# mcveanlab/mccortex

Hardware: AMD Instinct MI355X
Metric: k-mers/s inserted (build), k=31, 50M x 150bp synthetic reads (higher is better)
Workload: dtype u64

## Files before the change

### mccortex_amd/csrc/mcx_api.hip

```cpp
#include <hip/hip_runtime.h>

#include <stdarg.h>
#include <stdio.h>
#include <stdlib.h>
#include <string.h>
#include <cstring>

#include <rocprim/device/device_radix_sort.hpp>
#include <rocprim/device/device_scan.hpp>

#include <algorithm>
#include <array>
#include <cmath>
#include <memory>
#include <vector>
#include <thread>
#include <atomic>
#include <chrono>
#include <mutex>
#include <condition_variable>
#include <functional>

#include "../../include/mcx_gpu.h"
#include "mcx_kernels.h"
// ... 524 lines not shown
      case 2: if (one_) F<2, true>(__VA_ARGS__); else F<2, false>(__VA_ARGS__); break; \
      case 3: if (one_) F<3, true>(__VA_ARGS__); else F<3, false>(__VA_ARGS__); break; \
      default: if (one_) F<4, true>(__VA_ARGS__); else F<4, false>(__VA_ARGS__); break; \
    }                                                                                 \
  } while (0)
#define LAUNCH_W4(W_, KERNEL, ...)                                       \
  do {                                                                   \
    switch (W_) {                                                        \
      case 1: hipLaunchKernelGGL((KERNEL<1>), __VA_ARGS__); break;       \
      case 2: hipLaunchKernelGGL((KERNEL<2>), __VA_ARGS__); break;       \
      case 3: hipLaunchKernelGGL((KERNEL<3>), __VA_ARGS__); break;       \
      default: hipLaunchKernelGGL((KERNEL<4>), __VA_ARGS__); break;      \
    }                                                                    \
  } while (0)
#define NO_WIDE(g, what) do { if ((g) && (g)->W > 2) return fail(MCX_ERR_ARG, what " is not available for k > 63"); } while (0)

struct SpanGuard {
  mcx_graph *g; size_t idx; bool on;
  SpanGuard(mcx_graph *g_, const char *name) : g(g_), idx(0), on(g_ && g_->profile) {
    if (!on) return;
    mcx_graph::Span sp{name, nullptr, nullptr};
    (void)hipEventCreate(&sp.a); (void)hipEventCreate(&sp.b);
    (void)hipEventRecord(sp.a, g->stream);
    idx = g->spans.size();
    g->spans.push_back(sp);
  }
  ~SpanGuard() { if (on) (void)hipEventRecord(g->spans[idx].b, g->stream); }
};

static unsigned cl_grid(const mcx_graph *g, uint64_t items)
{
  return (unsigned)std::max<uint64_t>(1, std::min<uint64_t>((items + 255) / 256, (uint64_t)g->grid));
}
#define GRID_LAUNCH(NAME, ITEMS, ...)                                                            \
  do {                                                                                           \
    SpanGuard sp_(g, #NAME);                                                                     \
    hipLaunchKernelGGL(NAME, dim3(cl_grid(g, ITEMS)), dim3(256), 0, st, __VA_ARGS__);            \
    HIP_TRY(hipGetLastError());                                                                  \
  } while (0)
#define GRID_LAUNCH_W(NAME, ITEMS, ...)                                                          \
  do {                                                                                           \
    SpanGuard sp_(g, #NAME);                                                                     \
    LAUNCH_W4(g->W, NAME, dim3(cl_grid(g, ITEMS)), dim3(256), 0, st, __VA_ARGS__);               \
    HIP_TRY(hipGetLastError());                                                                  \
  } while (0)

static void phase_clock(const char *cmd, const char *what, double &t0)
{
  static const bool on = getenv("MCX_TIMING") != nullptr;
  if (!on) return;
  const double t = now_s();
  fprintf(stderr, "[timing]   %s %8.1f ms  %s\n", cmd, (t - t0) * 1e3, what);
  t0 = t;
}

template <class In> static int device_scan(hipStream_t st, const In *in, uint64_t *out, uint64_t cnt)
{
  size_t tmp_bytes = 0;
  HIP_TRY(rocprim::exclusive_scan(nullptr, tmp_bytes, in, out, (uint64_t)0, cnt, rocprim::plus<uint64_t>(), st));
  DevBuf<uint8_t> tmp;
  HIP_TRY(tmp.alloc(std::max<size_t>(tmp_bytes, 1)));
  HIP_TRY(rocprim::exclusive_scan((void *)tmp.p, tmp_bytes, in, out, (uint64_t)0, cnt, rocprim::plus<uint64_t>(), st));
  HIP_TRY(hipStreamSynchronize(st));
  return MCX_OK;
}
template <class In> static int scan_total(hipStream_t st, const In *in, uint64_t *out, uint64_t cnt, uint64_t *total)
{
  int rc = device_scan(st, in, out, cnt);
  if (rc != MCX_OK) return rc;
  HIP_TRY(hipMemcpy(total, out + cnt - 1, 8, hipMemcpyDeviceToHost));
  return MCX_OK;
}

static int sort_perm_scratch(hipStream_t st, uint64_t m, size_t *tmp_bytes)
{
  HIP_TRY(rocprim::radix_sort_pairs(nullptr, *tmp_bytes, (const uint64_t *)nullptr, (uint64_t *)nullptr, (uint64_t *)nullptr, (uint64_t *)nullptr, m, 0, 64, st));
  return MCX_OK;
}
template <class WordFn>
static int sort_perm_by_words(hipStream_t st, uint64_t m, int W, int top_bits, uint64_t *const keys[2], uint64_t *const perm[2], void *tmp,
                              size_t tmp_bytes, mcx_graph *span, WordFn word, uint64_t **out)
{
  uint64_t *cur = perm[0], *nxt = perm[1];
  for (int w = W - 1; w >= 0; w--) {
    const uint64_t *have = nullptr;
    int rc = word(w, w == W - 1, (const uint64_t *)cur, keys[1], &have);
    if (rc != MCX_OK) return rc;
    auto radix_sort_pass = [&](auto *in) {
      SpanGuard sp(span, "radix_sort_pairs");
      return rocprim::radix_sort_pairs(tmp, tmp_bytes, in, keys[0], cur, nxt, m, 0, w ? 64 : top_bits, st);
    };
    HIP_TRY(have ? radix_sort_pass(have) : radix_sort_pass(keys[1]));
    std::swap(cur, nxt);
  }
  *out = cur;
  return MCX_OK;
}

template <class K> static void allow_lds(K kernel, size_t bytes)
{
  (void)hipFuncSetAttribute(reinterpret_cast<const void *>(kernel), hipFuncAttributeMaxDynamicSharedMemorySize, (int)bytes);
}

static StreamArgs make_args(mcx_graph *g, const StreamLaunch &L)
{
  StreamArgs a;
  a.stream = L.stream; a.code = L.code; a.inv = L.inv; a.nbytes = L.nbytes; a.pos_lo = L.pos_lo; a.pos_hi = L.pos_hi;
  a.tile0 = L.pos_lo / kTile;
  a.ntiles = (L.pos_hi + kTile - 1) / kTile;
  a.k = g->k; a.ctr = g->d_ctr; a.flag = L.flag;
  return a;
}

template <int W, bool ONECOL> static void launch_direct_t(mcx_graph *g, const StreamLaunch &L, int colour)
{
  const StreamArgs a = make_args(g, L);
  const uint64_t nt = a.ntiles > a.tile0 ? a.ntiles - a.tile0 : 0;
  if (!nt) return;
  InsertSink<W, ONECOL> is{g->t, (uint32_t)colour};
  SpanGuard sp(g, "k_stream");
  const dim3 grid((unsigned)std::min<uint64_t>(nt, (uint64_t)g->grid));
  if (a.code) hipLaunchKernelGGL((k_stream<W, ONECOL, true>), grid, dim3(kThreads), 0, g->stream, a, is);
  else hipLaunchKernelGGL((k_stream<W, ONECOL, false>), grid, dim3(kThreads), 0, g->stream, a, is);
}

template <int W, bool ONECOL, bool FULL, int SH, bool PK>
static void launch_bin_stream_pk(mcx_graph *g, const StreamArgs &a, uint64_t nt, int colour, BinSpec bs, BinOut out)
{
  InsertSink<W, ONECOL> is{g->t, (uint32_t)colour};
  static bool once_dev[64] = {false};
  bool &once = once_dev[g->device & 63];
  if (!once) {
    allow_lds(k_stream_bin<W, ONECOL, 512, FULL, SH, PK>, sizeof(BinLds<W, 512, FULL>));
    allow_lds(k_stream_bin<W, ONECOL, 1024, FULL, SH, PK>, sizeof(BinLds<W, 1024, FULL>));
    allow_lds(k_stream_bin<W, ONECOL, kMaxBins, FULL, SH, PK>, sizeof(BinLds<W, kMaxBins, FULL>));
    once = true;
  }
  SpanGuard sp(g, "k_stream_bin");
  if constexpr (W == 1 && !FULL && SH == 0) {
    static const int fc_cap = [] { const char *e = getenv("MCX_STREAM_FC"); return e ? atoi(e) : 0; }();
    if (fc_cap && bs.nlocal <= 512) {
      const dim3 gridf((unsigned)std::min<uint64_t>(nt, (uint64_t)(g->grid_stream ? g->grid_stream : g->grid)));
#define MCX_FC_LAUNCH(CAPV, PRIVV) { \
        static bool once_f[64] = {false}; \
        if (!once_f[g->device & 63]) { allow_lds(k_stream_fc<ONECOL, PK, CAPV, PRIVV>, sizeof(FcLds<CAPV>)); once_f[g->device & 63] = true; } \
        hipLaunchKernelGGL((k_stream_fc<ONECOL, PK, CAPV, PRIVV>), gridf, dim3(kThreads), sizeof(FcLds<CAPV>), g->stream, a, bs, out, is); }
      if (bs.rep >= gridf.x && bs.rep > 8) MCX_FC_LAUNCH(10, true)
      else MCX_FC_LAUNCH(10, false)
#undef MCX_FC_LAUNCH
      return;
    }
    static const bool wide = [] { const char *e = getenv("MCX_STREAM_T"); return !e || atoi(e) == 512; }();
    if (wide && bs.nlocal <= 512) {
      using GeoW = Geo<512, 512 * kPosPerLane>;
      static bool once_w[64] = {false};
      if (!once_w[g->device & 63]) { allow_lds(k_stream_bin<W, ONECOL, 512, FULL, SH, PK, 512>, sizeof(BinLds<W, 512, FULL, GeoW>)); once_w[g->device & 63] = true; }
      const dim3 gridw((unsigned)std::min<uint64_t>((nt + 1) / 2, (uint64_t)(g->grid_stream ? g->grid_stream : g->grid)));
      hipLaunchKernelGGL((k_stream_bin<W, ONECOL, 512, FULL, SH, PK, 512>), gridw, dim3(512), sizeof(BinLds<W, 512, FULL, GeoW>), g->stream, a, bs, out, is);
      return;
    }
  }
  const dim3 grid((unsigned)std::min<uint64_t>(nt, (uint64_t)(g->grid_stream ? g->grid_stream : g->grid)));
  if (bs.nlocal <= 512)
    hipLaunchKernelGGL((k_stream_bin<W, ONECOL, 512, FULL, SH, PK>), grid, dim3(kThreads), sizeof(BinLds<W, 512, FULL>), g->stream, a, bs, out, is);
  else if (bs.nlocal <= 1024)
    hipLaunchKernelGGL((k_stream_bin<W, ONECOL, 1024, FULL, SH, PK>), grid, dim3(kThreads), sizeof(BinLds<W, 1024, FULL>), g->stream, a, bs, out, is);
  else
    hipLaunchKernelGGL((k_stream_bin<W, ONECOL, kMaxBins, FULL, SH, PK>), grid, dim3(kThreads), sizeof(BinLds<W, kMaxBins, FULL>), g->stream, a, bs, out, is);
}

template <int W, bool ONECOL, bool FULL, int SH>
static void launch_bin_stream_t(mcx_graph *g, const StreamLaunch &L, int colour, BinSpec bs, BinOut out)
{
  const StreamArgs a = make_args(g, L);
  const uint64_t nt = a.ntiles > a.tile0 ? a.ntiles - a.tile0 : 0;
  if (!nt) return;
  if (!FULL && a.code) launch_bin_stream_pk<W, ONECOL, FULL, SH, !FULL>(g, a, nt, colour, bs, out);
  else launch_bin_stream_pk<W, ONECOL, FULL, SH, false>(g, a, nt, colour, bs, out);
}

template <int W, bool ONECOL, bool IN_FULL, bool SHARD>
static void launch_bin_tuples_t(mcx_graph *g, TupleIn in, int colour, BinSpec bs, BinOut out)
{
  constexpr bool kWide = W == 1 && !IN_FULL;
  static const bool wide = kWide && [] { const char *e = getenv("MCX_SPLIT_T"); return !e || atoi(e) == 512; }();
  const bool use_wide = wide && bs.nlocal <= 1024;
  const bool use_huge = wide && !use_wide && bs.nlocal <= (uint32_t)kMaxBins;
  const uint64_t tile = use_huge ? 1024 * 16 : use_wide ? 512 * 16 : kTile;
  const uint64_t nchunks = (in.seg_cap + tile - 1) / tile * in.nseg;
  if (!nchunks) return;
  InsertSink<W, ONECOL> is{g->t, (uint32_t)colour};
  using GeoW = Geo<512, 512 * 16>;
  static bool once_dev[64] = {false};
  bool &once = once_dev[g->device & 63];
  if (!once) {
    allow_lds(k_tuples_bin<W, ONECOL, 512, IN_FULL, SHARD>, sizeof(BinLds<W, 512, false>));
    allow_lds(k_tuples_bin<W, ONECOL, 1024, IN_FULL, SHARD>, sizeof(BinLds<W, 1024, false>));
    allow_lds(k_tuples_bin<W, ONECOL, kMaxBins, IN_FULL, SHARD>, sizeof(BinLds<W, kMaxBins, false>));
    if constexpr (kWide) allow_lds(k_tuples_bin<W, ONECOL, 512, IN_FULL, SHARD, 512>, sizeof(BinLds<W, 512, false, GeoW>));
    if constexpr (kWide) allow_lds(k_tuples_bin<W, ONECOL, 1024, IN_FULL, SHARD, 512>, sizeof(BinLds<W, 1024, false, GeoW>));
    if constexpr (kWide) allow_lds(k_tuples_bin<W, ONECOL, kMaxBins, IN_FULL, SHARD, 1024>, sizeof(BinLds<W, kMaxBins, false, Geo<1024, 1024 * 16>>));
    once = true;
  }
  SpanGuard sp(g, "k_tuples_bin");
  const uint64_t gmax = (uint64_t)(g->grid_split ? g->grid_split : g->grid * 4);
  if constexpr (kWide) {
    if (use_huge) {
      using GeoH = Geo<1024, 1024 * 16>;
      const dim3 gridh((unsigned)std::min<uint64_t>(nchunks, g->grid_split ? gmax : gmax / 4));
      hipLaunchKernelGGL((k_tuples_bin<W, ONECOL, kMaxBins, IN_FULL, SHARD, 1024>), gridh, dim3(1024), sizeof(BinLds<W, kMaxBins, false, GeoH>), g->stream, in, bs, out, is, g->d_ctr);
      return;
    }
    if (use_wide) {
      const dim3 gridw((unsigned)std::min<uint64_t>(nchunks, g->grid_split ? gmax : gmax / 2));
      if (bs.nlocal <= 512)
        hipLaunchKernelGGL((k_tuples_bin<W, ONECOL, 512, IN_FULL, SHARD, 512>), gridw, dim3(512), sizeof(BinLds<W, 512, false, GeoW>), g->stream, in, bs, out, is, g->d_ctr);
      else
        hipLaunchKernelGGL((k_tuples_bin<W, ONECOL, 1024, IN_FULL, SHARD, 512>), gridw, dim3(512), sizeof(BinLds<W, 1024, false, GeoW>), g->stream, in, bs, out, is, g->d_ctr);
      return;
    }
  }
  const dim3 grid((unsigned)std::min<uint64_t>(nchunks, gmax));
  if (bs.nlocal <= 512)
    hipLaunchKernelGGL((k_tuples_bin<W, ONECOL, 512, IN_FULL, SHARD>), grid, dim3(kThreads), sizeof(BinLds<W, 512, false>), g->stream, in, bs, out, is, g->d_ctr);
  else if (bs.nlocal <= 1024)
    hipLaunchKernelGGL((k_tuples_bin<W, ONECOL, 1024, IN_FULL, SHARD>), grid, dim3(kThreads), sizeof(BinLds<W, 1024, false>), g->stream, in, bs, out, is, g->d_ctr);
  else
    hipLaunchKernelGGL((k_tuples_bin<W, ONECOL, kMaxBins, IN_FULL, SHARD>), grid, dim3(kThreads), sizeof(BinLds<W, kMaxBins, false>), g->stream, in, bs, out, is, g->d_ctr);
}
template <int W, bool ONECOL> static void launch_bin_region_stream(mcx_graph *g, const StreamLaunch &L, int colour, BinSpec bs, BinOut out)
{
  if (g->t.lbo) launch_bin_stream_t<W, ONECOL, false, 1>(g, L, colour, bs, out);
  else launch_bin_stream_t<W, ONECOL, false, 0>(g, L, colour, bs, out);
}
template <int W, bool ONECOL> static void launch_split_regions(mcx_graph *g, TupleIn in, int colour, BinSpec bs, BinOut out)
{ launch_bin_tuples_t<W, ONECOL, false, false>(g, in, colour, bs, out); }
template <int W, bool ONECOL> static void launch_bin_received(mcx_graph *g, TupleIn in, int colour, BinSpec bs, BinOut out)
{
  if (g->t.lbo) launch_bin_tuples_t<W, ONECOL, true, true>(g, in, colour, bs, out);
  else launch_bin_tuples_t<W, ONECOL, true, false>(g, in, colour, bs, out);
}

static uint64_t *l2_ptr(const mcx_graph *g, uint64_t off)
{
  if (g->l2_hi && off >= g->l2_hi_off) return g->l2_hi + (off - g->l2_hi_off) * g->cap2 * g->W;
  return g->l2_keys + off * g->cap2 * g->W;
}

template <int W, bool ONECOL, bool IDX32> static void launch_lds_insert_k(mcx_graph *g, int colour, uint32_t sub0, uint32_t nsub)
{
  const size_t lds = Sub<W>::kSlots * (W + 1) * 8 + LdsQueue<W>::kTuples * 8 * W;
  static bool once_dev[64] = {false};
  bool &once = once_dev[g->device & 63];
  if (!once) { allow_lds(k_lds_insert<W, ONECOL, IDX32>, lds); once = true; }
  BinOut bins{l2_ptr(g, g->l2_off), nullptr, g->l2_cnt + g->l2_off, g->cap2, nullptr, nullptr, nullptr, 0};
  SpanGuard sp(g, "k_lds_insert");
  hipLaunchKernelGGL((k_lds_insert<W, ONECOL, IDX32>), dim3((unsigned)std::min<uint64_t>(nsub, (uint64_t)(g->grid_insert ? g->grid_insert : g->grid * 4))),
                     dim3(LdsCfg<W>::kThreads), lds, g->stream, g->t, (uint32_t)colour, bins, sub0, nsub, g->d_ctr);
}

template <int W, bool ONECOL> static void launch_lds_insert_t(mcx_graph *g, int colour, uint32_t sub0, uint32_t nsub)
{
  if constexpr (W == 1 && ONECOL) {
    if (g->l2_idx32) return launch_lds_insert_k<W, ONECOL, true>(g, colour, sub0, nsub);
  }
  launch_lds_insert_k<W, ONECOL, false>(g, colour, sub0, nsub);
}

template <int W, bool ONECOL>
static void launch_insert_tuples_t(mcx_graph *g, int colour, const uint64_t *keys, const uint8_t *edges, uint64_t n, uint32_t only_own = 0)
{
  const int grid = (int)std::min<uint64_t>((n + kThreads * kBatch - 1) / (kThreads * kBatch), (uint64_t)g->grid);
  InsertSink<W, ONECOL> s{g->t, (uint32_t)colour};
  SpanGuard sp(g, "k_insert_tuples");
  hipLaunchKernelGGL((k_insert_tuples<W, ONECOL>), dim3(grid), dim3(kThreads), 0, g->stream, s, keys, edges, n, g->d_ctr, only_own);
}

static void free_defer(mcx_graph *g)
{
  (void)hipFree(g->l1_keys); (void)hipFree(g->l1_cnt);
  (void)hipFree(g->l2_base); (void)hipFree(g->l2_hi); (void)hipFree(g->l2_cnt);
  g->l1_keys = g->l2_keys = g->l2_base = g->l2_hi = nullptr; g->l1_cnt = g->l2_cnt = nullptr;
  g->cap1 = g->cap2 = 0;
  g->l2_regions = 0;
  g->set_colour.clear(); g->set_pending.clear();
}

__global__ __launch_bounds__(512) void k_l2_probe(uint64_t *keys, uint64_t cap, uint32_t nregions, uint32_t spb, uint32_t iters,
                                                  uint32_t jit_mask = 0 )
{
  const uint32_t region = blockIdx.x % nregions, blk = blockIdx.x / nregions, nblk = gridDim.x / nregions;
  const uint32_t w = threadIdx.x >> 6, l = threadIdx.x & 63u;
  for (uint32_t it = 0; it < iters; it++)
    for (uint32_t k = 0; k < spb / 32u; k++) {
      const uint32_t front = w * 4u + (l >> 4) + 32u * k;
      const uint32_t seg = region * spb + front;
      const uint64_t jit = ((seg * 0x9E3779B1u) >> 8) & jit_mask & ~15u;
      const uint64_t at = (uint64_t)seg * cap + jit + ((uint64_t)it * nblk + blk) * 16u + (l & 15u);
      if (jit + ((uint64_t)it * nblk + blk) * 16u + 16u <= cap) keys[at] = at;
    }
}

static uint64_t *l2_place(mcx_graph *g, size_t bytes, uint32_t nreg, int tries, float *ms_out)
{
  std::vector<uint64_t *> cand;
  std::vector<float> ms;
  hipEvent_t e0 = nullptr, e1 = nullptr;
  if (tries > 1 && (hipEventCreate(&e0) != hipSuccess || hipEventCreate(&e1) != hipSuccess)) { (void)hipGetLastError(); tries = 1; }
  const uint32_t iters = (uint32_t)std::max<uint64_t>(8, g->cap2 * g->W / 1024);
  for (int i = 0; i < std::max(tries, 1); i++) {
    if (i > 0) {
// ... 4105 lines not shown
```

### mccortex_amd/csrc/mcx_defer.h

```cpp
#pragma once
#include "mcx_kernels.h"

namespace mcx {

enum : int { BIN_OWNER = 0, BIN_GROUP = 1, BIN_SUBLOCAL = 2, BIN_GLOBAL = 3 };

struct BinSpec {
  int mode;
  uint32_t nparts;
  uint32_t nlocal;
  uint32_t rep;
  uint32_t nout;
  uint32_t seg_mod;
  uint32_t lb1;
  uint32_t region0;
};

__device__ __forceinline__ uint32_t out_seg(const BinSpec &bs, uint32_t ob0, uint32_t b)
{
  if (bs.mode == BIN_GLOBAL)
    return ((((b >> bs.lb1) * bs.rep + blockIdx.x % bs.rep) << bs.lb1) | (b & ((1u << bs.lb1) - 1u)));
  return ob0 + b;
}

struct BinOut {
  uint64_t *keys;
  uint8_t *edges;
  unsigned long long *counts;
  uint64_t cap;
  uint64_t *ov_keys;
  uint8_t *ov_edges;
  unsigned long long *ov_counts;
  uint64_t ov_cap;
};

#define MCX_LDS_AS __attribute__((address_space(3)))

#ifdef MCX_PHASES
__device__ unsigned long long g_phase[3][8];
#define MCX_PH_DECL unsigned long long ph_t = wall_clock64(), ph_acc[8] = {0, 0, 0, 0, 0, 0, 0, 0};
#define MCX_PH(i) { const unsigned long long n_ = wall_clock64(); ph_acc[i] += n_ - ph_t; ph_t = n_; }
#define MCX_PH_COUNT ph_acc[7]++;
#define MCX_PH_DUMP(kid) { if (threadIdx.x == 0) for (int i_ = 0; i_ < 8; i_++) atomicAdd(&g_phase[kid][i_], ph_acc[i_]); }
#else
#define MCX_PH_DECL
#define MCX_PH(i)
#define MCX_PH_COUNT
#define MCX_PH_DUMP(kid)
#endif
constexpr int kMaxBins = 2048;
constexpr uint64_t kQMask = (1ull << 56) - 1;

template <int W> __device__ __forceinline__ Kmer<W> tuple_pack(const Kmer<W> &q, uint32_t e)
{
  Kmer<W> t = q;
  t.w[0] |= (uint64_t)e << 56;
  return t;
}
template <int W> __device__ __forceinline__ Kmer<W> tuple_q(const Kmer<W> &t)
{
  Kmer<W> q = t;
  q.w[0] &= kQMask;
  return q;
}

constexpr int kRounds = 2;
constexpr int kStage = kTile / kRounds;

template <int T_, int TILE_, int R_ = kRounds> struct Geo {
  static constexpr int kT = T_, kTileG = TILE_, kRoundsG = R_, kStageG = TILE_ / R_;
};
using Geo256 = Geo<kThreads, kTile>;

template <int W, int NB, bool FULL, class G = Geo256> struct BinLds {
  using geo = G;
  uint64_t skey[G::kStageG * W];
  unsigned long long gbase[NB];
  uint32_t cnt[NB + 64];
  uint32_t rnk[NB + 64];
  uint32_t off[NB + 64];
  uint32_t wsum[G::kT / 64];
  uint16_t sbin[G::kStageG];
  uint8_t se[FULL ? G::kStageG : 16];
};

__device__ __forceinline__ uint32_t tid_now()
{
  uint32_t t = threadIdx.x;
  asm volatile("" : "+v"(t));
  return t;
}

template <int NB, int T = kThreads> struct BinRes { unsigned long long g0[(NB + T - 1) / T]; };

template <class LDS, int NB>
__device__ __forceinline__ void bin_reserve(LDS &L, const BinSpec &bs, const BinOut &out, uint32_t ob0, BinRes<NB, LDS::geo::kT> &res,
                                            bool trash_beyond = false)
{
  constexpr int kT = LDS::geo::kT;
  const int tid = threadIdx.x;
  __syncthreads();
  {
    constexpr int PERB = NB / kT;
    static_assert(NB % kT == 0, "bins per thread");
    uint32_t c[PERB], x = 0;
#pragma unroll
    for (int i = 0; i < PERB; i++) {
      const uint32_t b = (uint32_t)tid * PERB + i;
      c[i] = b < bs.nlocal ? L.cnt[b] : 0;
      x += c[i];
    }
    const uint32_t mine = x;
#pragma unroll
    for (int d = 1; d < 64; d <<= 1) {
      const uint32_t y = __shfl_up(x, d, 64);
      if ((tid & 63) >= d) x += y;
    }
    if ((tid & 63) == 63) L.wsum[tid >> 6] = x;
    __syncthreads();
    uint32_t before = 0, total = 0;
#pragma unroll
    for (int w = 0; w < kT / 64; w++) {
      const uint32_t ws = L.wsum[w];
      if (w < (tid >> 6)) before += ws;
      total += ws;
    }
    uint32_t o = before + x - mine;
#pragma unroll
    for (int i = 0; i < PERB; i++) {
      const uint32_t b = (uint32_t)tid * PERB + i;
      if (b < bs.nlocal) L.off[b] = o;
      o += c[i];
    }
    if (tid < 64) L.off[bs.nlocal + tid] = tid && trash_beyond ? (uint32_t)LDS::geo::kTileG : total;
  }
  __syncthreads();
#pragma unroll
  for (int q = 0; q < (NB + kT - 1) / kT; q++) {
    const uint32_t b = (uint32_t)q * kT + tid;
    res.g0[q] = 0;
    if (b < bs.nlocal) {
      const uint32_t c = L.cnt[b];
      if (c) res.g0[q] = atomicAdd(&out.counts[out_seg(bs, ob0, b)], (unsigned long long)c);
    }
  }
}

constexpr unsigned long long kDstMask = (1ULL << 48) - 1;

template <class LDS, int NB>
__device__ __forceinline__ void bin_commit(LDS &L, const BinSpec &bs, const BinOut &out, uint32_t ob0, const BinRes<NB, LDS::geo::kT> &res)
{
  constexpr int kT = LDS::geo::kT;
#pragma unroll
  for (int q = 0; q < (NB + kT - 1) / kT; q++) {
    const uint32_t b = (uint32_t)q * kT + threadIdx.x;
    if (b < bs.nlocal) {
      const uint32_t o0 = L.off[b], o1 = L.off[b + 1];
      const unsigned long long g0 = res.g0[q];
      const unsigned long long room = out.cap > g0 ? out.cap - g0 : 0;
      const uint32_t lim = o0 + (uint32_t)min((unsigned long long)(o1 - o0), room);
      const unsigned long long dst = ((unsigned long long)out_seg(bs, ob0, b) * out.cap + g0 - o0) & kDstMask;
      L.gbase[b] = dst | ((unsigned long long)lim << 48);
    }
  }
}

template <class LDS> __device__ __forceinline__ uint32_t bin_rank(LDS &L, uint32_t local)
{
  return L.off[local] + atomicAdd(&L.rnk[local], 1u);
}

template <int W, bool FULL, class LDS>
__device__ __forceinline__ void bin_place(LDS &L, int round, uint32_t p, uint32_t local, const Kmer<W> &t, uint32_t e)
{
  constexpr uint32_t kSt = LDS::geo::kStageG;
  if ((int)(p / kSt) != round) return;
  const uint32_t q = p % kSt;
  L.skey[q * W] = t.w[0];
  if (W == 2) L.skey[q * W + 1] = t.w[W - 1];
  L.sbin[q] = (uint16_t)local;
  if (FULL) L.se[q] = (uint8_t)e;
}

template <int W, bool ONECOL, bool FULL, int SH, class LDS>
__device__ __forceinline__ void bin_writeout(LDS &L, int round, const BinSpec &bs, const BinOut &out, uint32_t ob0,
                                             uint32_t region_of_seg, const InsertSink<W, ONECOL> &isink,
                                             uint32_t &novel, uint32_t &full)
{
  __syncthreads();
  const uint32_t n = L.off[bs.nlocal];
  constexpr uint32_t kSt = LDS::geo::kStageG;
  const uint32_t lo = (uint32_t)round * kSt;
  const uint32_t hi = min(n, lo + kSt);
  auto emit = [&](uint32_t p, uint32_t b, unsigned long long gb, uint64_t t0, uint64_t t1) {
    if (p < (uint32_t)(gb >> 48)) {
      const uint64_t at = (gb + p) & kDstMask;
      uint64_t *kd = out.keys + at * W;
      kd[0] = t0;
      if (W == 2) kd[1] = t1;
      if (FULL) out.edges[at] = L.se[p - lo];
    } else if (FULL || bs.mode == BIN_OWNER) {
      full = 2;
    } else {
      Kmer<W> tq;
      tq.w[0] = t0;
      if (W == 2) tq.w[W - 1] = t1;
      const uint32_t e = (uint32_t)(tq.w[0] >> 56);
      const Kmer<W> qq = tuple_q<W>(tq);
      const uint32_t lbq = lbq_of(isink.t);
      if (SH == 2) {
        const Kmer<W> key = key_unquot<W>(qq, lbq, b ^ mix_g(region_mix<W>(qq), lbq));
        const uint32_t owner = b >> bs.lb1;
        const unsigned long long pos = atomicAdd(&out.ov_counts[owner], 1ULL);
        if (pos < out.ov_cap) {
          uint64_t *kd = out.ov_keys + ((uint64_t)owner * out.ov_cap + pos) * W;
          kd[0] = key.w[0];
          if (W == 2) kd[1] = key.w[W - 1];
          out.ov_edges[(uint64_t)owner * out.ov_cap + pos] = (uint8_t)e;
        } else {
          const unsigned long long sp_cap = bs.region0 ? out.ov_counts[bs.nparts + 1] : 0;
          const unsigned long long sp = sp_cap ? atomicAdd(&out.ov_counts[bs.nparts], 1ULL) : 0;
          if (sp < sp_cap) {
            const uint64_t at = (uint64_t)bs.nparts * out.ov_cap + sp;
            uint64_t *kd = out.ov_keys + at * W;
            kd[0] = key.w[0];
            if (W == 2) kd[1] = key.w[W - 1];
            out.ov_edges[at] = (uint8_t)e;
          } else {
            full = 2;
          }
        }
      } else {
        table_mark_written(isink.t);
        table_count_fallback(isink.t);
        const uint32_t region = bs.mode == BIN_GROUP ? b : region_of_seg;
        const Kmer<W> key = key_unquot<W>(qq, lbq, r_of<W>(isink.t, region, qq));
        const uint64_t slot = key_slot<W>(isink.t, key);
        const uint64_t cur = *key_ptr_t<W, ONECOL>(isink.t, slot);
        probe_insert<W, ONECOL>(isink.t, key, slot, cur, 0, e, isink.col, novel, full);
      }
    }
  };
  for (uint32_t p = lo + threadIdx.x; p < hi; p += LDS::geo::kT) {
    const uint32_t q = p - lo;
    const uint32_t b = L.sbin[q];
    emit(p, b, L.gbase[b], L.skey[q * W], W == 2 ? L.skey[q * W + W - 1] : 0);
  }
  if (round + 1 < LDS::geo::kRoundsG) __syncthreads();
}

struct LaneWin { uint32_t a2, a1, a0, r2, r1, r0; };
__device__ __forceinline__ uint32_t pairrev32(uint32_t x)
{
  const uint32_t r = __builtin_bitreverse32(x);
  return ((r >> 1) & 0x55555555u) | ((r & 0x55555555u) << 1);
}
__device__ __forceinline__ LaneWin lane_win(const uint32_t *s_code, uint32_t pl, int k)
{
  LaneWin w;
  w.a2 = s_code[pl >> 4];
  w.a1 = s_code[(pl >> 4) + 1];
  w.a0 = s_code[(pl >> 4) + 2];
  const uint32_t c2 = pairrev32(~w.a0), c1 = pairrev32(~w.a1), c0 = pairrev32(~w.a2);
  const int t = 66 - 2 * k;
  if (t < 32) {
    w.r2 = (c2 << t) | (c1 >> (32 - t));
    w.r1 = (c1 << t) | (c0 >> (32 - t));
    w.r0 = c0 << t;
  } else {
    const uint64_t x = (((uint64_t)c1 << 32) | c0) << (t - 32);
    w.r2 = (uint32_t)(x >> 32);
    w.r1 = (uint32_t)x;
    w.r0 = 0;
  }
  return w;
}

template <int W, bool ONECOL>
__device__ __noinline__ void foreign_insert(const InsertSink<W, ONECOL> &isink, Kmer<W> key, uint32_t e,
                                            uint32_t &novel, uint32_t &full)
{
  table_mark_written(isink.t);
  table_count_foreign(isink.t);
  const uint64_t slot = key_slot<W>(isink.t, key);
  const uint64_t cur = *key_ptr_t<W, ONECOL>(isink.t, slot);
  probe_insert<W, ONECOL>(isink.t, key, slot, cur, 0, e, isink.col, novel, full);
}

template <int W, bool ONECOL, int NB, bool FULL, int SH, bool PK, int T = kThreads>
__global__ __launch_bounds__(T, (W == 1 ? 4 : 3)) void k_stream_bin(StreamArgs a_arg, BinSpec bs, BinOut out_arg,
                                                                  InsertSink<W, ONECOL> isink_arg)
{
  constexpr int H = T / kThreads;
  static_assert(T == kThreads || (T == 2 * kThreads && !FULL), "256 threads, or 512 for packed bins");
  __shared__ uint32_t s_code_h[H][kChunks + 4];
  __shared__ uint32_t s_inv_h[H][kChunks / 2 + 4];
  struct Cold { StreamArgs a; InsertSink<W, ONECOL> isink; };
  __shared__ Cold cold;
  if (threadIdx.x == 0) { cold.a = a_arg; cold.isink = isink_arg; }
  __syncthreads();
  const StreamArgs &a = cold.a;
  const BinOut &out = out_arg;
  const InsertSink<W, ONECOL> &isink = cold.isink;
  const uint64_t a_tile0 = a_arg.tile0, a_ntiles = a_arg.ntiles;
  const uint32_t t_lb1 = isink_arg.t.lb1, t_lbq = isink_arg.t.lb1 + isink_arg.t.lbo, t_part = isink_arg.t.part;
  extern __shared__ __attribute__((aligned(16))) unsigned char dyn_lds[];
  using LDS = BinLds<W, NB, FULL, Geo<T, T * kPosPerLane>>;
  LDS &L = *reinterpret_cast<LDS *>(dyn_lds);

  const int tid0 = threadIdx.x & (kThreads - 1);
  const uint64_t half0 = (uint64_t)(threadIdx.x / kThreads);
  const int k = a_arg.k;
  uint32_t n_kmers = 0, n_contigs = 0, n_novel = 0, full = 0;
  const uint64_t top_mask = (W == 1) ? (~0ULL >> (64 - 2 * k)) : (~0ULL >> (128 - 2 * k));
  const int first_shift = (W == 1) ? (2 * k - 2) : (2 * k - 66);
  const uint32_t ob0 = (blockIdx.x % bs.rep) * bs.nout;

  TileSrc pre;
  pre.a = make_uint4(0, 0, 0, 0); pre.b = make_uint4(0, 0, 0, 0);
  {
    const uint64_t t0 = a_tile0 + (uint64_t)blockIdx.x * H + half0;
    if (t0 < a_ntiles) tile_fetch<PK>(a_arg, t0, tid0, pre);
  }
  MCX_PH_DECL
  for (uint64_t tile_b = a_tile0 + (uint64_t)blockIdx.x * H; tile_b < a_ntiles; tile_b += (uint64_t)gridDim.x * H) {
    const int tid_blk = (int)tid_now();
    const int tid = tid_blk & (kThreads - 1);
    const uint64_t tile = tile_b + (uint64_t)(tid_blk / kThreads);
    const bool have_tile = H == 1 || tile < a_ntiles;
    uint32_t *s_code = s_code_h[H == 1 ? 0 : tid_blk / kThreads];
    uint32_t *s_inv = s_inv_h[H == 1 ? 0 : tid_blk / kThreads];
    MCX_PH(6) MCX_PH_COUNT
    tile_stage<PK>(a_arg, pre, tid, s_code, s_inv);
    for (uint32_t b = tid_blk; b < bs.nlocal + 64; b += T) { L.cnt[b] = 0; L.rnk[b] = 0; }
    if (tid < 4) { s_code[kChunks + tid] = 0; s_inv[kChunks / 2 + tid] = 0xFFFFFFFFu; }
    {
      const uint64_t tn = tile + (uint64_t)gridDim.x * H;
      if (tn < a_ntiles) tile_fetch<PK>(a_arg, tn, tid, pre);
    }
    __syncthreads();
    MCX_PH(0)

    const uint32_t pl = 16u * (uint32_t)(tid + 1);
    const uint64_t Vh = inv_win64(s_inv, pl);
    const uint64_t Vl = (W == 2) ? inv_win64(s_inv, pl + 64) : 0;
    const uint32_t prev_chunk_inv = (s_inv[(pl - 1) >> 5] >> (31 - ((pl - 1) & 31))) & 1u;
    uint32_t range = have_tile ? 0xFFFFu : 0u;
    if (have_tile) {
      const uint64_t plo = a.pos_lo, phi = a.pos_hi, T0 = tile * kTile;
      if (T0 < plo || T0 + kTile > phi) {
        const uint64_t P0 = T0 + 16ull * (uint64_t)tid;
        const int j_lo = plo > P0 ? (int)min((uint64_t)kPosPerLane, plo - P0) : 0;
        const int j_hi = phi > P0 ? (int)min((uint64_t)kPosPerLane, phi - P0) : 0;
        range = ((0x10000u >> j_lo) - 1u) & ~((0x10000u >> j_hi) - 1u);
      }
    }
    uint32_t ok16, nok16, pok16;
    {
      uint64_t Mh = Vh, Ml = Vl;
      for (int c = 1; c < k;) {
        const int s = min(c, k - c);
        if (W == 2) Mh |= (Mh << s) | (Ml >> (64 - s));
        else Mh |= Mh << s;
        if (W == 2) Ml |= Ml << s;
        c += s;
      }
      ok16 = ~(uint32_t)(Mh >> 48) & range;
      const int sh = 112 - k;
      const uint64_t nx = sh >= 64 ? (Vh >> (sh - 64)) : ((Vh << (64 - sh)) | (W == 2 ? (Vl >> sh) : 0));
      nok16 = ~(uint32_t)nx & 0xFFFFu;
      pok16 = ~((prev_chunk_inv << 15) | (uint32_t)(Vh >> 49)) & 0xFFFFu;
    }

    Kmer<W> tk[kPosPerLane];
    uint32_t tle[kPosPerLane];
    const uint32_t trash = bs.nlocal + 1u + ((uint32_t)tid_blk & 31u);
    n_kmers += __popc(ok16);
    n_contigs += __popc(ok16 & ~pok16);
    {
      const uint32_t own = s_code[pl >> 4];
      const uint32_t before = s_code[(pl - 1) >> 4] & 3u;
      const uint32_t lbq = t_lbq;
      const uint32_t qmask = (1u << lbq) - 1u, lmask = (1u << t_lb1) - 1u;
      Kmer<W> fw, rc;
      uint64_t feed;
      LaneWin lw;
      if (W == 1) {
        lw = lane_win(s_code, pl, k);
        feed = code_win64(s_code, pl + (uint32_t)k);
      } else {
        const uint64_t hi = code_win64(s_code, pl), lo = code_win64(s_code, pl + 32);
        const int s = 128 - 2 * k;
        fw.w[0] = hi >> s;
        fw.w[W - 1] = (lo >> s) | (hi << (64 - s));
        rc = revcomp<W>(fw, k);
        feed = code_win64(s_code, pl + (uint32_t)k);
      }
      const uint32_t feed32 = (uint32_t)(feed >> 32);
      uint32_t arr_prev = 0;
      const uint32_t key_sh = 64u - 2u * (uint32_t)k;
      const uint32_t mix_sh = (32u - lbq) & 31u;
#pragma unroll
      for (int j = 0; j < kPosPerLane; j++) {
        const uint32_t prev_nuc = j == 0 ? before : ((own >> (32 - 2 * j)) & 3u);
        const uint32_t nuc_next = (feed32 >> (30 - 2 * j)) & 3u;
        const uint32_t valid = 0u - ((ok16 >> (15 - j)) & 1u);
        const uint32_t nb = (nok16 >> (15 - j)) & 1u, pb = (pok16 >> (15 - j)) & 1u;
        uint32_t o, local;
        Kmer<W> key;
        uint64_t sel = 0;
        if (W == 1) {
          const uint32_t fh = j ? __builtin_amdgcn_alignbit(lw.a2, lw.a1, 32 - 2 * j) : lw.a2;
          const uint32_t fl = j ? __builtin_amdgcn_alignbit(lw.a1, lw.a0, 32 - 2 * j) : lw.a1;
          const uint32_t rh = j < 15 ? __builtin_amdgcn_alignbit(lw.r2, lw.r1, 2 + 2 * j) : lw.r2;
          const uint32_t rl = j < 15 ? __builtin_amdgcn_alignbit(lw.r1, lw.r0, 2 + 2 * j) : lw.r1;
          const uint64_t f = ((uint64_t)fh << 32) | fl, r = ((uint64_t)rh << 32) | rl;
          o = f < r ? 0u : 1u;
          sel = f < r ? f : r;
          key.w[0] = sel >> key_sh;
        } else {
          key = canonical<W>(fw, rc, o);
        }
        const uint32_t o4 = o << 2;
        const uint32_t e = (nb << (nuc_next | o4)) | (pb << ((prev_nuc ^ 7u) ^ o4));
        if (FULL) {
          uint32_t h2;
          kmer_hash<W>(key, 0, &h2);
          local = owner_of(h2, bs.nparts);
          tk[j] = key;
          local = (local & valid) | (trash & ~valid);
          tle[j] = local | (e << 24);
        } else {
          uint32_t G;
          Kmer<W> q;
          if (W == 1) {
            const uint64_t kk = sel >> key_sh;
            q.w[0] = kk >> lbq;
            G = ((uint32_t)kk ^ (region_mix<W>(q) >> mix_sh)) & qmask;
          } else {
            uint32_t r;
            q = key_quot<W>(key, lbq, r);
            G = r ^ mix_g(region_mix<W>(q), lbq);
          }
          local = SH == 1 ? (G & lmask) : G;
          tk[j] = tuple_pack<W>(q, e);
          if (SH == 1 && valid && (G >> t_lb1) != t_part) {
            foreign_insert<W, ONECOL>(isink, key, e, n_novel, full);
            local = trash;
          }
          local = (local & valid) | (trash & ~valid);
          tle[j] = local;
        }
        const uint32_t arr_now = atomicAdd(&L.cnt[local], 1u);
        if (j > 0) { tle[j - 1] |= arr_prev << 12; asm volatile("" : "+v"(tle[j - 1])); }
        arr_prev = arr_now;
        if (j == kPosPerLane - 1) tle[j] |= arr_now << 12;
        if (W == 1) asm volatile("" : "+v"(tle[j]), "+v"(tk[j].w[0]));
        else asm volatile("" : "+v"(tle[j]), "+v"(tk[j].w[0]), "+v"(tk[j].w[W - 1]));
        if (W == 2) {
          fw.w[0] = ((fw.w[0] << 2) | (fw.w[W - 1] >> 62)) & top_mask;
          fw.w[W - 1] = (fw.w[W - 1] << 2) | nuc_next;
          rc.w[W - 1] = (rc.w[W - 1] >> 2) | (rc.w[0] << 62);
          rc.w[0] = (rc.w[0] >> 2) | ((uint64_t)(3u - nuc_next) << first_shift);
        }
      }
    }
    MCX_PH(1)
    BinRes<NB, T> res;
    bin_reserve<LDS, NB>(L, bs, out, ob0, res, !FULL);
    MCX_PH(2)
#pragma unroll
    for (int j = 0; j < kPosPerLane; j++) {
      tle[j] += L.off[tle[j] & 0xfffu] << 12;
      if ((j & 3) == 3) asm volatile("" : "+v"(tle[j - 3]), "+v"(tle[j - 2]), "+v"(tle[j - 1]), "+v"(tle[j]));
    }
    bin_commit<LDS, NB>(L, bs, out, ob0, res);
    MCX_PH(3)
    for (int round = 0; round < kRounds; round++) {
#pragma unroll
      for (int j = 0; j < kPosPerLane; j++)
        bin_place<W, FULL, LDS>(L, round, FULL ? (tle[j] >> 12) & 0xfffu : tle[j] >> 12, tle[j] & 0xfffu, tk[j], tle[j] >> 24);
      bin_writeout<W, ONECOL, FULL, SH, LDS>(L, round, bs, out, ob0, 0, isink, n_novel, full);
      if (round == 0) { MCX_PH(4) } else { MCX_PH(5) }
    }
  }
  MCX_PH_DUMP(0)

  block_add(&a.ctr->kmers, n_kmers);
  block_add(&a.ctr->contigs, n_contigs);
  block_add(&a.ctr->novel, n_novel);
  if (full == 1) a.ctr->full = 1;
  if (full == 2) a.ctr->bin_over = 1;
  if (a.flag && n_contigs) *a.flag = 1;
}

struct TupleIn {
  const uint64_t *keys;
  const uint8_t *edges;
  const unsigned long long *counts;
  uint64_t seg_cap;
  uint32_t nseg;
  uint32_t seg_group, seg_stride;
  uint32_t set_rep;
  uint8_t set_map[32];
};
__device__ __forceinline__ uint64_t tuple_seg_phys(const TupleIn &in, uint32_t seg)
{
  uint32_t q = seg / in.seg_group;
  if (in.set_rep) q = (uint32_t)in.set_map[q / in.set_rep] * in.set_rep + q % in.set_rep;
  return (uint64_t)q * in.seg_stride + seg % in.seg_group;
}

template <int W, bool ONECOL, int NB, bool IN_FULL, bool SHARD, int T = kThreads, int R = kRounds, int P = 16>
__global__ __launch_bounds__(T, (W == 1 || T > kThreads ? 4 : 3)) void k_tuples_bin(TupleIn in, BinSpec bs, BinOut out,
                                                                         InsertSink<W, ONECOL> isink_arg, Counters *ctr)
{
  extern __shared__ __attribute__((aligned(16))) unsigned char dyn_lds[];
  using LDS = BinLds<W, NB, false, Geo<T, T * P, R>>;
  constexpr int kThreads = T, kTile = T * P;
  LDS &L = *reinterpret_cast<LDS *>(dyn_lds);
  __shared__ InsertSink<W, ONECOL> isink;
  if (threadIdx.x == 0) isink = isink_arg;
  __syncthreads();
  const uint32_t t_spb = isink_arg.t.spb, t_lb1 = isink_arg.t.lb1, t_lbq = isink_arg.t.lb1 + isink_arg.t.lbo, t_part = isink_arg.t.part;
  const int tid = threadIdx.x;
  uint32_t n_novel = 0, full = 0;
  const uint64_t chunks_per_seg = (in.seg_cap + kTile - 1) / kTile;
  const bool xcd = bs.mode == BIN_SUBLOCAL && gridDim.x % 8 == 0 && bs.seg_mod % 8 == 0 && in.nseg % bs.seg_mod == 0;
  const uint32_t group = xcd ? blockIdx.x % 8 : 0;
  const uint32_t nseg_g = xcd ? in.nseg / 8 : in.nseg;
  constexpr uint32_t kWin = 2;
  const uint32_t bins_g = xcd ? bs.seg_mod / 8 : 1;
  const uint32_t reps = xcd ? in.nseg / bs.seg_mod : 1;
  const uint32_t win_segs = kWin * reps;
  const uint32_t nwin = (bins_g + kWin - 1) / kWin;
  const uint64_t nchunks = xcd ? (uint64_t)nwin * chunks_per_seg * win_segs : chunks_per_seg * nseg_g;
  const uint64_t v0 = xcd ? blockIdx.x / 8 : blockIdx.x, vstep = xcd ? gridDim.x / 8 : gridDim.x;
  const uint32_t lmask = (1u << t_lb1) - 1u;
  MCX_PH_DECL
  for (uint64_t v = v0; v < nchunks; v += vstep) {
    uint32_t seg;
    uint64_t start;
    if (xcd) {
      const uint64_t per_win = chunks_per_seg * win_segs;
      const uint32_t win = (uint32_t)(v / per_win);
      const uint64_t rem = v % per_win;
      const uint32_t s = (uint32_t)(rem % win_segs);
      const uint32_t rgi = win * kWin + s % kWin;
      if (rgi >= bins_g) continue;
      seg = (s / kWin) * bs.seg_mod + group + 8 * rgi;
      start = (rem / win_segs) * kTile;
    } else {
      seg = (uint32_t)(v % nseg_g);
      start = (v / nseg_g) * kTile;
    }
    const uint64_t pseg = tuple_seg_phys(in, seg);
    uint64_t cnt = in.counts ? (uint64_t)in.counts[pseg] : in.seg_cap;
    if (cnt > in.seg_cap) cnt = in.seg_cap;
    if (start >= cnt) continue;
    const uint32_t n = (uint32_t)min((uint64_t)kTile, cnt - start);
    const uint32_t lregion = bs.mode == BIN_SUBLOCAL ? seg % bs.seg_mod : 0;
    const uint32_t region = bs.region0 + lregion;
    const uint32_t ob0 = (bs.mode == BIN_SUBLOCAL ? lregion * t_spb : 0) + (blockIdx.x % bs.rep) * bs.nout;
    MCX_PH(6) MCX_PH_COUNT
    __syncthreads();
    for (uint32_t b = tid; b < bs.nlocal + 64; b += kThreads) { L.cnt[b] = 0; L.rnk[b] = 0; }
    __syncthreads();
    MCX_PH(0)
    const uint32_t trash = bs.nlocal + 1u + ((uint32_t)tid & 31u);
    const uint64_t *kin = in.keys + (pseg * in.seg_cap + start) * W;
    const uint8_t *ein = IN_FULL ? in.edges + pseg * in.seg_cap + start : nullptr;
    constexpr int PER = kTile / kThreads;
    Kmer<W> tk[PER];
    uint32_t ev[IN_FULL ? PER : 1], loc[PER];
    uint32_t okm = 0;
    const bool vec16 = !IN_FULL && (((uintptr_t)in.keys & 15u) == 0) && (W == 2 || (in.seg_cap & 1u) == 0);
    if (vec16) {
      const ulonglong2 *kin2 = reinterpret_cast<const ulonglong2 *>(kin);
#pragma unroll
      for (int q = 0; q < PER; q += (W == 1 ? 2 : 1)) {
        const uint32_t p = (uint32_t)(q / (W == 1 ? 2 : 1)) * kThreads + tid;
        const uint32_t i = W == 1 ? 2 * p : p;
        tk[q].w[0] = 0; tk[q + (W == 1 ? 1 : 0)].w[W - 1] = 0;
        if (i < n) {
          const ulonglong2 x = kin2[p];
          okm |= 1u << q;
          if (W == 1) {
            tk[q].w[0] = x.x;
            tk[q + (W == 1 ? 1 : 0)].w[0] = x.y;
            if (i + 1 < n) okm |= 2u << q;
          } else {
            tk[q].w[0] = x.x;
            tk[q].w[W - 1] = x.y;
          }
        }
      }
    } else {
#pragma unroll
    for (int q = 0; q < PER; q++) {
      const uint32_t i = (uint32_t)q * kThreads + tid;
      if (i < n) okm |= 1u << q;
      tk[q].w[0] = 0; if (W == 2) tk[q].w[W - 1] = 0;
      if (IN_FULL) ev[q] = 0;
      if (i < n) {
        tk[q].w[0] = kin[(uint64_t)i * W];
        if (W == 2) tk[q].w[W - 1] = kin[(uint64_t)i * W + 1];
        if (IN_FULL) ev[q] = ein[i];
      }
    }
    }
#pragma unroll
    for (int q = 0; q < PER; q++) {
      const uint32_t i = (uint32_t)q * kThreads + tid;
      uint32_t hb;
      if (IN_FULL) {
        uint32_t r;
        const uint32_t lbq = t_lbq;
        const Kmer<W> key = tk[q];
        const Kmer<W> qq = key_quot<W>(key, lbq, r);
        const uint32_t G = r ^ mix_g(region_mix<W>(qq), lbq);
        hb = 0;
        loc[q] = G & lmask;
        tk[q] = tuple_pack<W>(qq, ev[q]);
        if (SHARD && (okm >> q & 1u) && (G >> t_lb1) != t_part) {
          foreign_insert<W, ONECOL>(isink, key, ev[q], n_novel, full);
          okm &= ~(1u << q);
        }
      } else {
        hb = sub_hash<W>(tuple_q<W>(tk[q]));
        loc[q] = __umulhi(hb, t_spb);
      }
      if (loc[q] >= bs.nlocal) loc[q] = bs.nlocal - 1;
      loc[q] = (okm >> q & 1u) ? loc[q] : trash;
      atomicAdd(&L.cnt[loc[q]], 1u);
      (void)i;
    }
// ... 524 lines not shown
```

Before: 105.7 billion.

## Use larger staging buffer in wide stream kernel and skip second round when unneeded

Gives the 512-thread stream-bin kernel its own LDS layout with a larger staging area (13*512 entries) and no rank array. The tile's binned k-mers are placed in a first stage covering most of the tile, and a second round runs only when the tile's total count exceeds that stage. This removes a barrier and a round of placement and writeout for most tiles. The layout is sized so two blocks still fit in the CU's LDS, which a static_assert checks. The cost is a different round split and more LDS per block.

```diff
diff --git a/mccortex_amd/csrc/mcx_api.hip b/mccortex_amd/csrc/mcx_api.hip
--- a/mccortex_amd/csrc/mcx_api.hip
+++ b/mccortex_amd/csrc/mcx_api.hip
@@ -700,11 +700,11 @@
     }
     static const bool wide = [] { const char *e = getenv("MCX_STREAM_T"); return !e || atoi(e) == 512; }();
     if (wide && bs.nlocal <= 512) {
-      using GeoW = Geo<512, 512 * kPosPerLane>;
+      using LdsW = StreamLdsWide<W, 512>;
       static bool once_w[64] = {false};
-      if (!once_w[g->device & 63]) { allow_lds(k_stream_bin<W, ONECOL, 512, FULL, SH, PK, 512>, sizeof(BinLds<W, 512, FULL, GeoW>)); once_w[g->device & 63] = true; }
+      if (!once_w[g->device & 63]) { allow_lds(k_stream_bin<W, ONECOL, 512, FULL, SH, PK, 512>, sizeof(LdsW)); once_w[g->device & 63] = true; }
       const dim3 gridw((unsigned)std::min<uint64_t>((nt + 1) / 2, (uint64_t)(g->grid_stream ? g->grid_stream : g->grid)));
-      hipLaunchKernelGGL((k_stream_bin<W, ONECOL, 512, FULL, SH, PK, 512>), gridw, dim3(512), sizeof(BinLds<W, 512, FULL, GeoW>), g->stream, a, bs, out, is);
+      hipLaunchKernelGGL((k_stream_bin<W, ONECOL, 512, FULL, SH, PK, 512>), gridw, dim3(512), sizeof(LdsW), g->stream, a, bs, out, is);
       return;
     }
   }
diff --git a/mccortex_amd/csrc/mcx_defer.h b/mccortex_amd/csrc/mcx_defer.h
--- a/mccortex_amd/csrc/mcx_defer.h
+++ b/mccortex_amd/csrc/mcx_defer.h
@@ -69,8 +69,13 @@
 
 template <int T_, int TILE_, int R_ = kRounds> struct Geo {
   static constexpr int kT = T_, kTileG = TILE_, kRoundsG = R_, kStageG = TILE_ / R_;
+  static constexpr bool kDynG = false;
 };
 using Geo256 = Geo<kThreads, kTile>;
+template <int T_, int TILE_, int STAGE_> struct GeoDyn {
+  static constexpr int kT = T_, kTileG = TILE_, kStageG = STAGE_, kRoundsG = (TILE_ + STAGE_ - 1) / STAGE_;
+  static constexpr bool kDynG = true;
+};
 
 template <int W, int NB, bool FULL, class G = Geo256> struct BinLds {
   using geo = G;
@@ -82,6 +87,18 @@
   uint32_t wsum[G::kT / 64];
   uint16_t sbin[G::kStageG];
   uint8_t se[FULL ? G::kStageG : 16];
+};
+
+constexpr int kStageWide = 13 * 512;
+template <int W, int NB> struct StreamLdsWide {
+  using geo = GeoDyn<2 * kThreads, 2 * kTile, kStageWide>;
+  uint64_t skey[geo::kStageG * W];
+  unsigned long long gbase[NB];
+  uint32_t cnt[NB + 64];
+  uint32_t off[NB + 64];
+  uint32_t wsum[geo::kT / 64];
+  uint16_t sbin[geo::kStageG];
+  uint8_t se[16];
 };
 
 __device__ __forceinline__ uint32_t tid_now()
@@ -247,7 +264,17 @@
     const uint32_t b = L.sbin[q];
     emit(p, b, L.gbase[b], L.skey[q * W], W == 2 ? L.skey[q * W + W - 1] : 0);
   }
-  if (round + 1 < LDS::geo::kRoundsG) __syncthreads();
+  if (!LDS::geo::kDynG && round + 1 < LDS::geo::kRoundsG) __syncthreads();
+}
+
+template <int W, class LDS>
+__device__ __forceinline__ void bin_place_at(LDS &L, uint32_t lo, uint32_t span, uint32_t p, uint32_t local, const Kmer<W> &t)
+{
+  const uint32_t q = p - lo;
+  if (q >= span) return;
+  L.skey[q * W] = t.w[0];
+  if (W == 2) L.skey[q * W + 1] = t.w[W - 1];
+  L.sbin[q] = (uint16_t)local;
 }
 
 struct LaneWin { uint32_t a2, a1, a0, r2, r1, r0; };
@@ -306,7 +333,10 @@
   const uint64_t a_tile0 = a_arg.tile0, a_ntiles = a_arg.ntiles;
   const uint32_t t_lb1 = isink_arg.t.lb1, t_lbq = isink_arg.t.lb1 + isink_arg.t.lbo, t_part = isink_arg.t.part;
   extern __shared__ __attribute__((aligned(16))) unsigned char dyn_lds[];
-  using LDS = BinLds<W, NB, FULL, Geo<T, T * kPosPerLane>>;
+  using LDS = std::conditional_t<T == 2 * kThreads, StreamLdsWide<W, NB>, BinLds<W, NB, FULL, Geo<T, T * kPosPerLane>>>;
+  static_assert(!LDS::geo::kDynG || W != 1 || NB != 512 ||
+                2 * (sizeof(LDS) + sizeof(s_code_h) + sizeof(s_inv_h) + sizeof(Cold)) <= 160 * 1024,
+                "two blocks of the wide stream kernel fit the CU's 160 KiB of LDS");
   LDS &L = *reinterpret_cast<LDS *>(dyn_lds);
 
   const int tid0 = threadIdx.x & (kThreads - 1);
@@ -333,7 +363,10 @@
     uint32_t *s_inv = s_inv_h[H == 1 ? 0 : tid_blk / kThreads];
     MCX_PH(6) MCX_PH_COUNT
     tile_stage<PK>(a_arg, pre, tid, s_code, s_inv);
-    for (uint32_t b = tid_blk; b < bs.nlocal + 64; b += T) { L.cnt[b] = 0; L.rnk[b] = 0; }
+    for (uint32_t b = tid_blk; b < bs.nlocal + 64; b += T) {
+      L.cnt[b] = 0;
+      if constexpr (!LDS::geo::kDynG) L.rnk[b] = 0;
+    }
     if (tid < 4) { s_code[kChunks + tid] = 0; s_inv[kChunks / 2 + tid] = 0xFFFFFFFFu; }
     {
       const uint64_t tn = tile + (uint64_t)gridDim.x * H;
@@ -475,14 +508,33 @@
       tle[j] += L.off[tle[j] & 0xfffu] << 12;
       if ((j & 3) == 3) asm volatile("" : "+v"(tle[j - 3]), "+v"(tle[j - 2]), "+v"(tle[j - 1]), "+v"(tle[j]));
     }
-    bin_commit<LDS, NB>(L, bs, out, ob0, res);
-    MCX_PH(3)
-    for (int round = 0; round < kRounds; round++) {
-#pragma unroll
-      for (int j = 0; j < kPosPerLane; j++)
-        bin_place<W, FULL, LDS>(L, round, FULL ? (tle[j] >> 12) & 0xfffu : tle[j] >> 12, tle[j] & 0xfffu, tk[j], tle[j] >> 24);
-      bin_writeout<W, ONECOL, FULL, SH, LDS>(L, round, bs, out, ob0, 0, isink, n_novel, full);
-      if (round == 0) { MCX_PH(4) } else { MCX_PH(5) }
+    if constexpr (LDS::geo::kDynG) {
+      constexpr uint32_t kSt = LDS::geo::kStageG, kTl = LDS::geo::kTileG;
+      static_assert(LDS::geo::kRoundsG == 2 && !FULL, "at most one round after the first");
+      const uint32_t n = __builtin_amdgcn_readfirstlane(L.off[bs.nlocal]);
+      MCX_PH(3)
+#pragma unroll
+      for (int j = 0; j < kPosPerLane; j++) bin_place_at<W, LDS>(L, 0, kSt, tle[j] >> 12, tle[j] & 0xfffu, tk[j]);
+      bin_commit<LDS, NB>(L, bs, out, ob0, res);
+      bin_writeout<W, ONECOL, FULL, SH, LDS>(L, 0, bs, out, ob0, 0, isink, n_novel, full);
+      MCX_PH(4)
+      if (n > kSt) {
+        __syncthreads();
+#pragma unroll
+        for (int j = 0; j < kPosPerLane; j++) bin_place_at<W, LDS>(L, kSt, kTl - kSt, tle[j] >> 12, tle[j] & 0xfffu, tk[j]);
+        bin_writeout<W, ONECOL, FULL, SH, LDS>(L, 1, bs, out, ob0, 0, isink, n_novel, full);
+        MCX_PH(5)
+      }
+    } else {
+      bin_commit<LDS, NB>(L, bs, out, ob0, res);
+      MCX_PH(3)
+      for (int round = 0; round < kRounds; round++) {
+#pragma unroll
+        for (int j = 0; j < kPosPerLane; j++)
+          bin_place<W, FULL, LDS>(L, round, FULL ? (tle[j] >> 12) & 0xfffu : tle[j] >> 12, tle[j] & 0xfffu, tk[j], tle[j] >> 24);
+        bin_writeout<W, ONECOL, FULL, SH, LDS>(L, round, bs, out, ob0, 0, isink, n_novel, full);
+        if (round == 0) { MCX_PH(4) } else { MCX_PH(5) }
+      }
     }
   }
   MCX_PH_DUMP(0)
```

New measurement: 107.2 billion, median of 6. 1.4% higher.
